# Lightbrite88/Argon_Monte_Carlo

Hardware: AMD Instinct MI355X
Metric: particle-steps/sec (higher is better)
Workload: dtype f64; 1 GPU; cube_1e5; geometry=cube, n_particles=100000, n_per_gpu=100000, parallelism=single GPU

## Files before the change

### argon_monte_carlo_amd/csrc/amc_api.hip

```cpp
#include <memory>
#include <type_traits>

#include "amc_host.h"

int amc_fail(amc_ctx *c, int code, const char *fmt, ...)
{
    char buf[512];
    va_list ap;
    va_start(ap, fmt);
    vsnprintf(buf, sizeof buf, fmt, ap);
    va_end(ap);
    if (c) c->err = buf;
    return code;
}

static thread_local std::string g_create_err;

void amc_prof_begin(amc_ctx *c, int kclass)
{
    if (!c->profiling) return;
    if (c->ev_used == c->ev_pool.size()) {
        hipEvent_t a, b;
        (void)ctx_event(c, &a, hipEventDefault);
        (void)ctx_event(c, &b, hipEventDefault);
// ... 272 lines not shown
    AMC_HIP(c, dalloc(c, &c->d_od, 16));
    AMC_HIP(c, hipMemsetAsync(c->d_od, 0, 16 * sizeof(int), c->stream));
    if (palloc(c, &c->h_pin, (size_t)4 << 20, hipHostMallocDefault) == hipSuccess) c->h_pin_bytes = (size_t)4 << 20;
    return AMC_OK;
}

extern "C" {

int amc_abi_version(void) { return AMC_ABI_VERSION; }

const char *amc_last_error(const amc_ctx *ctx) { return ctx ? ctx->err.c_str() : g_create_err.c_str(); }

const char *amc_kernel_name(int k)
{
    static const char *names[AMC_K_COUNT] = {"drift_walls", "bin_count", "bin_scan",     "bin_scatter", "detect",  "resolve",
                                             "bounds",      "validate",  "resolve_more", "commit",      "clusters_wide", "fixup",
                                             "fields"};
    return (k >= 0 && k < AMC_K_COUNT) ? names[k] : "?";
}

void amc_destroy(amc_ctx *c)
{
    if (!c) return;
    hipSetDevice(c->device);
    hipStreamSynchronize(c->stream);
    ctx_free_since(c, 0);
    delete c;
}

int amc_create(amc_ctx **out, const amc_params *p)
{
    if (!out || !p) { g_create_err = "null argument"; return AMC_ERR_INVALID; }
    *out = nullptr;
    if (p->struct_size != (int32_t)sizeof(amc_params)) {
        g_create_err = "amc_params.struct_size mismatch (ABI)";
        return AMC_ERR_INVALID;
    }
    if (p->n < 0 || p->n > 0x7fffffffLL || !(p->collision_range > 0) || !(p->argon_mass > 0) || p->geometry < 0 ||
        p->geometry > AMC_GEOM_PORE_ENERGISED) {
        g_create_err = "invalid amc_params (n, collision_range, argon_mass or geometry)";
        return AMC_ERR_INVALID;
    }
    int ndev = 0;
    if (hipGetDeviceCount(&ndev) != hipSuccess || ndev <= 0 || p->device < 0 || p->device >= ndev) {
        g_create_err = "no usable HIP device (libargonmc has no CPU fallback)";
        return AMC_ERR_NO_DEVICE;
    }
    amc_ctx *c = new (std::nothrow) amc_ctx();
    if (!c) { g_create_err = "out of host memory"; return AMC_ERR_INVALID; }
    c->P = *p;
    c->device = p->device;
    c->n = p->n; c->hi = p->n;
    c->keep_prior = (p->reserved0 & 1) != 0;
    read_env(c);
    std::unique_ptr<amc_ctx, void (*)(amc_ctx *)> guard(c, [](amc_ctx *x) { g_create_err = x->err; amc_destroy(x); });
    AMC_HIP(c, hipSetDevice(c->device));
    AMC_HIP(c, ctx_stream(c, &c->own_stream));
    c->stream = c->own_stream;
    c->allpairs = (p->geometry == AMC_GEOM_CELL) || (p->detect_mode != 1 && c->n <= c->allpairs_max_n);
    c->detect_ap = c->allpairs || p->detect_mode == 2;
    if (p->geometry == AMC_GEOM_CELL && p->detect_mode == 1) {
        return amc_fail(c, AMC_ERR_INVALID, "AMC_GEOM_CELL has no cell grid: detect_mode must be 0 or 2");
    }
    int rc;
    if ((rc = alloc_state(c)) || (rc = alloc_grid_lists(c)) || (rc = alloc_resolve_ws(c)) || (rc = alloc_outputs(c)) ||
        (rc = alloc_host_words(c)))
        return rc;
    if (c->debug_resolve) {
        AMC_HIP(c, dalloc(c, &c->d_dbg, 128 + 128 * 512));
        AMC_HIP(c, hipMemsetAsync(c->d_dbg, 0, sizeof(long long) * (128 + 128 * 512), c->stream));
        { const long long big = 0x7fffffffffffffffLL; AMC_HIP(c, hipMemcpyAsync(c->d_dbg + 28, &big, sizeof big, hipMemcpyHostToDevice, c->stream)); }
    }
    AMC_HIP(c, hipStreamSynchronize(c->stream));
    *out = guard.release();
    return AMC_OK;
}

int amc_set_stream(amc_ctx *c, void *hip_stream)
{
    if (!c) return AMC_ERR_INVALID;
    hipSetDevice(c->device);
    amc_prof_collect(c);
    if (c->stream) hipStreamSynchronize(c->stream);
    c->stream = hip_stream ? (hipStream_t)hip_stream : c->own_stream;
    return AMC_OK;
}

int amc_use_null_stream(amc_ctx *c)
{
    if (!c) return AMC_ERR_INVALID;
    hipSetDevice(c->device);
    amc_prof_collect(c);
    if (c->stream) hipStreamSynchronize(c->stream);
    c->stream = nullptr;
    return AMC_OK;
}

int amc_synchronize(amc_ctx *c)
{
    if (!c) return AMC_ERR_INVALID;
    AMC_HIP(c, hipSetDevice(c->device));
    AMC_HIP(c, hipStreamSynchronize(c->stream));
    return AMC_OK;
}

int amc_upload(amc_ctx *c, const double *x, const double *y, const double *z, const double *vx, const double *vy,
               const double *vz, const double *dist, const double *dist_x, const double *dist_y, const double *dist_z,
               const uint8_t *full_path)
{
    if (!c) return AMC_ERR_INVALID;
    AMC_HIP(c, hipSetDevice(c->device));
    { int rc_ = amc_flush(c); if (rc_) return rc_; }
    c->step.lists_age = -1;
    const size_t nb = sizeof(double) * (size_t)c->n;
    const double *src[] = {x, y, z, vx, vy, vz, dist, dist_x, dist_y, dist_z};
    double *dst[] = {c->S.x, c->S.y, c->S.z, c->S.vx, c->S.vy, c->S.vz, c->S.d, c->S.dx, c->S.dy, c->S.dz};
    for (int k = 0; k < 10; k++)
        if (src[k] && nb) AMC_HIP(c, hipMemcpyAsync(dst[k], src[k], nb, hipMemcpyHostToDevice, c->stream));
    if (full_path && c->n) AMC_HIP(c, hipMemcpyAsync(c->S.flag, full_path, (size_t)c->n, hipMemcpyHostToDevice, c->stream));
    { int rc_ = amc_publish_velocities(c); if (rc_) return rc_; }
    AMC_HIP(c, hipStreamSynchronize(c->stream));
    c->uploaded = true;
    return AMC_OK;
}

int amc_publish_velocities(amc_ctx *c)
{
    if (!c->kin_vpub || c->n <= 0) return AMC_OK;
    const size_t nb = sizeof(double) * (size_t)c->n;
    const double *src[3] = {c->S.vx, c->S.vy, c->S.vz};
    for (int e = 0; e < 3; e++)
        AMC_HIP(c, hipMemcpyAsync(c->kin_vpub + (size_t)e * (size_t)c->n, src[e], nb, hipMemcpyDeviceToDevice, c->stream));
    return AMC_OK;
}

int amc_download(amc_ctx *c, double *x, double *y, double *z, double *vx, double *vy, double *vz, double *dist,
                 double *dist_x, double *dist_y, double *dist_z, uint8_t *full_path)
{
    if (!c) return AMC_ERR_INVALID;
    AMC_HIP(c, hipSetDevice(c->device));
    { int rc_ = amc_flush(c); if (rc_) return rc_; }
    const size_t nb = sizeof(double) * (size_t)c->n;
    double *dst[] = {x, y, z, vx, vy, vz, dist, dist_x, dist_y, dist_z};
    double *src[] = {c->S.x, c->S.y, c->S.z, c->S.vx, c->S.vy, c->S.vz, c->S.d, c->S.dx, c->S.dy, c->S.dz};
    for (int k = 0; k < 10; k++)
        if (dst[k] && nb) AMC_HIP(c, hipMemcpyAsync(dst[k], src[k], nb, hipMemcpyDeviceToHost, c->stream));
    if (full_path && c->n) AMC_HIP(c, hipMemcpyAsync(full_path, c->S.flag, (size_t)c->n, hipMemcpyDeviceToHost, c->stream));
    AMC_HIP(c, hipStreamSynchronize(c->stream));
    return AMC_OK;
}

int amc_download_prior(amc_ctx *c, double *px, double *py, double *pz)
{
    if (!c) return AMC_ERR_INVALID;
    if (!c->keep_prior) return amc_fail(c, AMC_ERR_STATE, "prior_*_vals are only kept when amc_params.reserved0 bit0 is set");
    AMC_HIP(c, hipSetDevice(c->device));
    const size_t nb = sizeof(double) * (size_t)c->n;
    if (px && nb) AMC_HIP(c, hipMemcpyAsync(px, c->S.px, nb, hipMemcpyDeviceToHost, c->stream));
    if (py && nb) AMC_HIP(c, hipMemcpyAsync(py, c->S.py, nb, hipMemcpyDeviceToHost, c->stream));
    if (pz && nb) AMC_HIP(c, hipMemcpyAsync(pz, c->S.pz, nb, hipMemcpyDeviceToHost, c->stream));
    AMC_HIP(c, hipStreamSynchronize(c->stream));
    return AMC_OK;
}

int amc_paths_pending(amc_ctx *c, size_t *n)
{
    if (!c || !n) return AMC_ERR_INVALID;
    AMC_HIP(c, hipSetDevice(c->device));
    amc_dev_counters now;
    int rc = amc_read_counters(c, &now);
    if (rc) return rc;
    *n = std::min<size_t>(now.path_count, c->out.cap);
    return AMC_OK;
}

int amc_drain_paths(amc_ctx *c, amc_path_record *out, size_t cap, size_t *n)
{
    if (!c || !n) return AMC_ERR_INVALID;
    size_t pending;
    int rc = amc_paths_pending(c, &pending);
    if (rc) return rc;
    if (pending > cap) return amc_fail(c, AMC_ERR_CAPACITY, "amc_drain_paths: %zu records pending, buffer holds %zu", pending, cap);
    if (pending) AMC_HIP(c, hipMemcpyAsync(out, c->d_rec, sizeof(amc_path_record) * pending, hipMemcpyDeviceToHost, c->stream));
    unsigned int zero = 0;
    AMC_HIP(c, hipMemcpyAsync(&c->d_cnt->path_count, &zero, sizeof zero, hipMemcpyHostToDevice, c->stream));
    AMC_HIP(c, hipStreamSynchronize(c->stream));
    *n = pending;
    return AMC_OK;
}

int amc_histograms(amc_ctx *c, uint64_t *counts, uint64_t *n_paths_total)
{
    if (!c) return AMC_ERR_INVALID;
    AMC_HIP(c, hipSetDevice(c->device));
    if (counts) {
        if (!c->d_hist) return amc_fail(c, AMC_ERR_STATE, "histograms disabled (hist_bins == 0)");
    }
    { int rc_ = amc_settle_commit(c); if (rc_) return rc_; }
    std::vector<uint64_t> banks;
    if (counts) {
        banks.resize((size_t)4 * c->out.nbins * AMC_COUNTER_BANKS);
        AMC_HIP(c, hipMemcpyAsync(banks.data(), c->d_hist, sizeof(uint64_t) * banks.size(), hipMemcpyDeviceToHost, c->stream));
    }
    amc_dev_counters now;
    int rc = amc_read_counters(c, &now);
    if (rc) return rc;
    if (counts) {
        const size_t m = (size_t)4 * c->out.nbins;
        for (size_t k = 0; k < m; k++) counts[k] = 0;
        for (int b = 0; b < AMC_COUNTER_BANKS; b++)
            for (size_t k = 0; k < m; k++) counts[k] += banks[(size_t)b * m + k];
    }
    if (n_paths_total) *n_paths_total = now.n_paths_total;
    return AMC_OK;
}

int amc_reset_outputs(amc_ctx *c)
{
    if (!c) return AMC_ERR_INVALID;
    AMC_HIP(c, hipSetDevice(c->device));
    { int rc_ = amc_settle_commit(c); if (rc_) return rc_; }
    if (c->d_hist) AMC_HIP(c, hipMemsetAsync(c->d_hist, 0, sizeof(uint64_t) * 4 * c->out.nbins * AMC_COUNTER_BANKS, c->stream));
    AMC_HIP(c, hipMemsetAsync(c->d_cnt, 0, sizeof(amc_dev_counters), c->stream));
    AMC_HIP(c, hipMemsetAsync(c->d_banks, 0, sizeof(amc_counter_bank) * AMC_COUNTER_BANKS, c->stream));
    AMC_HIP(c, hipStreamSynchronize(c->stream));
    memset(&c->h_prev, 0, sizeof c->h_prev);
    c->out.step = 0;
    return AMC_OK;
}

int amc_pairwise_cell(amc_ctx *c, int64_t n_cell, double *continue_path, double *continue_x_path, double *continue_y_path,
                      double *continue_z_path, uint8_t *has_collided, double *x, double *y, double *z, double *vx,
                      double *vy, double *vz, double *out_paths, size_t cap, size_t *n_paths, int64_t *n_collisions)
{
    if (!c) return AMC_ERR_INVALID;
    if (c->P.geometry != AMC_GEOM_CELL) return amc_fail(c, AMC_ERR_STATE, "amc_pairwise_cell needs an AMC_GEOM_CELL context");
    if (n_cell < 0 || n_cell > c->n) return amc_fail(c, AMC_ERR_INVALID, "n_cell %lld exceeds the context capacity %lld", (long long)n_cell, (long long)c->n);
    AMC_HIP(c, hipSetDevice(c->device));
    const int64_t n_full = c->n;
    c->n = n_cell; c->lo = 0; c->hi = n_cell;
    int rc = amc_upload(c, x, y, z, vx, vy, vz, continue_path, continue_x_path, continue_y_path, continue_z_path, has_collided);
    amc_step_stats st;
    memset(&st, 0, sizeof st);
    size_t pending = 0;
    if (!rc) {
        size_t dummy;
        rc = amc_paths_pending(c, &dummy);
    }
    if (!rc) rc = amc_timestep(c, 0.0, &st);
    if (!rc) rc = amc_download(c, x, y, z, vx, vy, vz, continue_path, continue_x_path, continue_y_path, continue_z_path, has_collided);
    if (!rc) rc = amc_paths_pending(c, &pending);
    if (!rc && pending) {
        std::vector<amc_path_record> rec(pending);
        size_t got = 0;
        rc = amc_drain_paths(c, rec.data(), pending, &got);
        if (!rc) {
            std::sort(rec.begin(), rec.begin() + got, [](const amc_path_record &a, const amc_path_record &b) {
                if (a.step != b.step) return a.step < b.step;
                if (a.i != b.i) return a.i < b.i;
                if (a.j != b.j) return a.j < b.j;
                return a.which < b.which;
            });
            if (got > cap) rc = amc_fail(c, AMC_ERR_CAPACITY, "out_paths holds %zu paths, %zu were completed", cap, got);
            else if (out_paths)
                for (size_t k = 0; k < got; k++) {
                    out_paths[0 * cap + k] = rec[k].total; out_paths[1 * cap + k] = rec[k].px;
                    out_paths[2 * cap + k] = rec[k].py; out_paths[3 * cap + k] = rec[k].pz;
                }
            pending = got;
        }
    }
    if (n_paths) *n_paths = pending;
    if (n_collisions) *n_collisions = st.n_pp;
    c->n = n_full; c->lo = 0; c->hi = n_full;
    return rc;
}

int amc_profile(amc_ctx *c, int enable)
{
    if (!c) return AMC_ERR_INVALID;
    hipSetDevice(c->device);
    amc_prof_collect(c);
    c->profiling = enable != 0;
    return AMC_OK;
}

int amc_overlap_stats(amc_ctx *c, int64_t *out)
{
    if (!c || !out) return AMC_ERR_INVALID;
    AMC_HIP(c, hipSetDevice(c->device));
    amc_dev_counters now;
    int rc = amc_read_counters(c, &now);
    if (rc) return rc;
    out[0] = c->ovl_steps; out[1] = now.n_refiled; out[2] = c->overlap_mode; out[3] = c->max_extra;
    out[4] = c->od_ordered_launches; out[5] = c->od_steps; out[6] = c->od_stalls; out[7] = c->od_stalls_last;
    return AMC_OK;
}

int amc_kernel_times(amc_ctx *c, double *total_ms, int64_t *launches)
{
    if (!c) return AMC_ERR_INVALID;
    hipSetDevice(c->device);
    amc_prof_collect(c);
    if (c->d_dbg) {
        long long h[128];
        hipMemcpy(h, c->d_dbg, sizeof h, hipMemcpyDeviceToHost);
        const double n = h[11] > 0 ? (double)h[11] : 1.0;
        fprintf(stderr, "[amc k_resolve phases, us/launch] count-left %.1f claim %.1f | rounds: collect %.1f pairs %.1f clusters>=3: sort+load %.1f emulate %.1f | overlay %.1f validate %.1f commit %.1f | rounds %.2f cand %.1f complex-members %.2f launches %lld (idle hand-over only %lld)\n",
                h[0] / n / 100.0, h[1] / n / 100.0, h[6] / n / 100.0, h[7] / n / 100.0, h[2] / n / 100.0, h[3] / n / 100.0, h[14] / n / 100.0, h[4] / n / 100.0, h[5] / n / 100.0,
                h[8] / n, h[9] / n, h[10] / n, h[11], h[12]);
        fprintf(stderr, "[amc host candidate count] %d (what the next launch plan is chosen from)\n", c->h_host_ncand ? (int)*c->h_host_ncand : -1);
        if (h[12] > 0)
            fprintf(stderr, "[amc k_resolve idle hand-over, us/launch] entry -> counts read %.2f, -> hand-over written %.2f, -> through the barrier %.2f (%lld launches)\n",
                    h[16] / (double)h[12] / 100.0, h[17] / (double)h[12] / 100.0, h[18] / (double)h[12] / 100.0, h[12]);
        {
            std::vector<long long> wv((size_t)128 * 512);
            hipMemcpy(wv.data(), c->d_dbg + 128, sizeof(long long) * wv.size(), hipMemcpyDeviceToHost);
            long long s[128] = {0}, longest = 0;
            for (int w = 0; w < 512; w++) {
                for (int e = 3; e < 128; e++) if (e != 4) s[e] += wv[(size_t)128 * w + e];
                longest = std::max(longest, wv[(size_t)128 * w + 4]);
            }
            const double nl = h[25] > 0 ? (double)h[25] : 1.0;
            static const char *cn[8] = {"pair", "3-cluster", "4+-cluster", "not owner", "pair+again", "3-cluster+again", "4+-cluster+again", "not owner+again"};
            static const char *pn[12] = {"graph", "walk", "reserve", "small: after emulate", "pair emulate | by the wave: emulate", "publish", "grid probe", "first hop", "particles", "set-up", "overlay probe", "small: prepare"};
            fprintf(stderr, "[amc k_clusters_wide] working waves %lld in %lld launches; launch span (first working wave in -> last out) %.2f us, last out -> ordered workgroup in %.2f us, longest wave ever %.2f us\n",
                    s[3], h[25], h[27] / nl / 100.0, h[26] / nl / 100.0, longest / 100.0);
            fprintf(stderr, "[three-particle path of lane 0] %lld times, %lld continued from the pair's hit; loads + slots %.2f us, emulation %.2f us\n", s[5], s[6],
                    s[7] / (double)std::max<long long>(1, s[5]) / 100.0, s[124] / (double)std::max<long long>(1, s[5]) / 100.0);
            fprintf(stderr, "[pair-wave lifetimes, 2.5 us buckets]");
            for (int k = 0; k < 8; k++) fprintf(stderr, " %lld", s[24 + k]);
            fprintf(stderr, "\n");
            for (int k = 0; k < 8; k++) {
                if (!s[16 + k]) continue;
                fprintf(stderr, "[amc k_clusters_wide %-16s %7lld waves, %5.1f us]", cn[k], s[16 + k], s[8 + k] / (double)s[16 + k] / 100.0);
                for (int e = 0; e < 12; e++) fprintf(stderr, " %s %.2f", pn[e], s[32 + 12 * k + e] / (double)s[16 + k] / 100.0);
                fprintf(stderr, "\n");
            }
        }
    }
    for (int k = 0; k < AMC_K_COUNT; k++) {
        if (total_ms) total_ms[k] = c->k_ms[k];
        if (launches) launches[k] = c->k_launches[k];
    }
    return AMC_OK;
}

}
```

### argon_monte_carlo_amd/csrc/amc_grid.hip

```cpp
#include <stdlib.h>

#include "amc_grid_dev.h"

#define AMC_CR2_INFLATE (1.0 + 1.0e-9)

__global__ __launch_bounds__(256) void k_bin_lists(const double *__restrict__ x, const double *__restrict__ y,
                                                   const double *__restrict__ z, long long n, amc_grid G, amc_lists B,
                                                   amc_dev_counters *cnt, amc_ovl V)
{
    const long long p = (long long)blockIdx.x * blockDim.x + threadIdx.x;
    if (p >= n) return;
    if (V.skip_epoch && (unsigned int)(V.adj_head[p] >> 32) == V.skip_epoch) return;
    bool outside = false;
    amc_list_insert(G, B, (int)p, x[p], y[p], z[p], &outside);
    if (outside) atomicOr(&cnt->flags, 8ULL);
}

struct amc_adj {
    unsigned long long *head;
    int4 *rec;
    int4 *sd;
    int4 *sl_meta;
    int *sl_hits, *ev_gen;
    unsigned int epoch;
    unsigned long long *mark;
};

AMC_DEV int amc_push_candidate(int a, int b, int max_cand, amc_dev_counters *cnt, const amc_adj &D)
{
    const unsigned int k = atomicAdd(&cnt->cand_count, 1u);
    if (k < (unsigned)max_cand) {
        const int hi = a > b ? a : b, lo = a > b ? b : a;
        int4 r;
        r.x = hi; r.y = lo; r.z = -1; r.w = -1;
        if (D.head) {
            const unsigned long long mine = ((unsigned long long)D.epoch << 32) | (unsigned long long)k;
            const unsigned long long oi = atomicExch(&D.head[hi], mine), oj = atomicExch(&D.head[lo], mine);
            r.z = ((unsigned int)(oi >> 32) == D.epoch) ? (int)(unsigned int)(oi & 0xffffffffULL) : -1;
            r.w = ((unsigned int)(oj >> 32) == D.epoch) ? (int)(unsigned int)(oj & 0xffffffffULL) : -1;
            auto mark = [&](int kd) {
                const unsigned long long old = atomicExch(&D.mark[kd], mine);
                if ((unsigned int)(old >> 32) == D.epoch) D.mark[kd] = ((unsigned long long)D.epoch << 32) | AMC_MARK_MULTI;
            };
            if (r.z >= 0) mark(r.z);
            if (r.w >= 0) mark(r.w);
        }
        D.rec[k] = r;
        D.sd[k] = make_int4(-1, -1, 0, 0);
        if (D.head) {
            D.sl_meta[2 * k] = make_int4(-1, 2 * (int)k, 0, 0);
            D.sl_meta[2 * k + 1] = make_int4(-1, 2 * (int)k + 1, 0, 0);
            atomicAnd(&D.sl_hits[2 * k], 0);
            atomicAnd(&D.sl_hits[2 * k + 1], 0);
            *(int4 *)&D.ev_gen[4 * k] = make_int4(0, 0, 0, 0);
        }
        return (int)k;
    }
    atomicOr(&cnt->flags, 1ULL);
    return -1;
}

AMC_DEV void amc_detect_node(const amc_grid &G, const amc_lists &B, int node, double cr2i, double cr_probe, int max_cand,
                             amc_dev_counters *cnt, const amc_adj &D, const int *od_stall = nullptr, int od_tick = 0)
{
    const int stalled = od_stall ? *od_stall : 0;
    amc_rec me_r = B.rec[node];
    const int live = (B.node_of && node < B.n) ? B.node_of[node] : node;
    if (stalled && od_tick > stalled) return;
    if (me_r.x != me_r.x) {
        if (live == node) return;
        node = live;
        me_r = B.rec[node];
        if (me_r.x != me_r.x) return;
    }
    const int me_p = amc_node_particle(B, node);
    double3 me;
    amc_rec_pos(G, me_r, me.x, me.y, me.z);
    auto found_pair = [&](int q) { amc_push_candidate(me_p, amc_node_particle(B, q), max_cand, cnt, D); };
    int q[9];
    q[0] = amc_rec_next(me_r);
    {
        int ocx, ocy, ocz;
        amc_grid_coords(G, me.x, me.y, me.z, ocx, ocy, ocz);
        const int c_own = amc_grid_cell(G, ocx, ocy, ocz, nullptr);
        int c_lo[4], c_hi[4];
        const int nc = amc_grid_box_ranges(G, me.x, me.y, me.z, cr_probe, c_lo, c_hi);
        int cell[8];
#pragma unroll
        for (int k = 0; k < 4; k++)
#pragma unroll
            for (int t = 0; t < 2; t++) {
                const int c = c_lo[k < nc ? k : 0] + t;
                cell[2 * k + t] = (k < nc && c <= c_hi[k < nc ? k : 0] && c < c_own) ? c : -1;
            }
        unsigned long long hv[8];
#pragma unroll
        for (int e = 0; e < 8; e++) hv[e] = (cell[e] >= 0) ? B.head[cell[e]] : 0ULL;
#pragma unroll
        for (int e = 0; e < 8; e++)
            q[1 + e] = (cell[e] >= 0 && (unsigned int)(hv[e] >> 32) == B.epoch) ? (int)(unsigned int)(hv[e] & 0xffffffffULL) : -1;
    }
    for (;;) {
        bool live = false;
#pragma unroll
        for (int e = 0; e < 9; e++) live |= q[e] >= 0;
        if (!live) break;
        amc_rec o[9];
#pragma unroll
        for (int e = 0; e < 9; e++)
            if (q[e] >= 0) o[e] = B.rec[q[e]];
#pragma unroll
        for (int e = 0; e < 9; e++)
            if (q[e] >= 0) {
                double ox, oy, oz;
                amc_rec_pos(G, o[e], ox, oy, oz);
                const double ex = ox - me.x, ey = oy - me.y, ez = oz - me.z;
                if (ex * ex + ey * ey + ez * ez < cr2i) found_pair(q[e]);
                q[e] = amc_rec_next(o[e]);
            }
    }
}

#ifndef AMC_DETECT_MINW
#define AMC_DETECT_MINW 4
#endif
__global__ __launch_bounds__(256, AMC_DETECT_MINW) void k_detect_lists(amc_grid G, amc_lists B, long long n, double cr2i, double cr_probe,
                                                      int max_cand, amc_dev_counters *cnt, amc_adj D, const int *extra_count,
                                                      int max_extra, const int *od_stall, int od_tick, int *wctl_rearm)
{
    const long long nb = (n + blockDim.x - 1) / blockDim.x;
    if ((long long)blockIdx.x < nb) {
        const long long p = (long long)blockIdx.x * blockDim.x + threadIdx.x;
        if (p < n) amc_detect_node(G, B, (int)p, cr2i, cr_probe, max_cand, cnt, D, od_stall, od_tick);
        if (wctl_rearm && p == 0 && !(*od_stall && od_tick > *od_stall)) {
            amc_resolve_ctl *wc = (amc_resolve_ctl *)wctl_rearm;
            for (int b = 0; b < 16; b++) wctl_rearm[32 + b] = 0;
            wc->nslots = 0; wc->nhist = 0; wc->nedges = 0; wc->nfp = 0; wc->ovf = 0; wc->dirty = 0; wc->nclusters = 0;
            wc->changed = 0; wc->active = 0; wc->cur_round = 1;
        }
        return;
    }
    if (!extra_count) return;
    int ne = *extra_count;
    if (ne > max_extra) ne = max_extra;
    const int stride = (int)((gridDim.x - nb) * blockDim.x);
    for (int e = (int)((blockIdx.x - nb) * blockDim.x + threadIdx.x); e < ne; e += stride)
        amc_detect_node(G, B, (int)n + e, cr2i, cr_probe, max_cand, cnt, D, od_stall, od_tick);
}

__global__ __launch_bounds__(256) void k_detect_own(amc_grid G, amc_lists B, long long lo, long long hi, double cr2i,
                                                    double cr_probe, int *__restrict__ out, int cap, amc_dev_counters *cnt)
{
    const long long p = lo + (long long)blockIdx.x * blockDim.x + threadIdx.x;
    if (p >= hi) return;
    amc_rec me_r = B.rec[p];
    const int live = B.node_of ? B.node_of[p] : (int)p;
    if (me_r.x != me_r.x) {
        if (live == (int)p) return;
        me_r = B.rec[live];
        if (me_r.x != me_r.x) return;
    }
    double3 me;
    amc_rec_pos(G, me_r, me.x, me.y, me.z);
    int c_lo[4], c_hi[4];
    const int nc = amc_grid_box_ranges(G, me.x, me.y, me.z, cr_probe, c_lo, c_hi);
    int q[8];
    unsigned long long hv[8];
#pragma unroll
    for (int k = 0; k < 4; k++)
#pragma unroll
        for (int t = 0; t < 2; t++) {
            const int c = c_lo[k < nc ? k : 0] + t;
            const bool on = k < nc && c <= c_hi[k < nc ? k : 0];
            hv[2 * k + t] = on ? B.head[c] : 0ULL;
            q[2 * k + t] = on ? 0 : -1;
        }
#pragma unroll
    for (int e = 0; e < 8; e++)
        q[e] = (q[e] == 0 && (unsigned int)(hv[e] >> 32) == B.epoch) ? (int)(unsigned int)(hv[e] & 0xffffffffULL) : -1;
    for (;;) {
        bool live = false;
#pragma unroll
        for (int e = 0; e < 8; e++) live |= q[e] >= 0;
        if (!live) break;
        amc_rec o[8];
#pragma unroll
        for (int e = 0; e < 8; e++)
            if (q[e] >= 0) o[e] = B.rec[q[e]];
#pragma unroll
        for (int e = 0; e < 8; e++)
            if (q[e] >= 0) {
                double ox, oy, oz;
                amc_rec_pos(G, o[e], ox, oy, oz);
                const double ex = ox - me.x, ey = oy - me.y, ez = oz - me.z;
                const int pq = amc_node_particle(B, q[e]);
                if (pq < (int)p && ex * ex + ey * ey + ez * ez < cr2i) {
                    const int k = atomicAdd(&out[0], 1);
                    if (k < cap) { out[2 + 2 * k] = (int)p; out[3 + 2 * k] = pq; }
                    else atomicOr(&cnt->flags, 1ULL);
                }
                q[e] = amc_rec_next(o[e]);
            }
    }
}

__global__ __launch_bounds__(256) void k_ingest_candidates(const int *__restrict__ blocks, int world, int block_ints, int cap,
                                                           int max_cand, amc_dev_counters *cnt, amc_adj D, int *__restrict__ own)
{
    const int gtid = blockIdx.x * blockDim.x + threadIdx.x, gstride = gridDim.x * blockDim.x;
    for (int r = 0; r < world; r++) {
        const int *b = blocks + (size_t)r * block_ints;
        int nr = b[0];
        if (nr > cap) {
            nr = cap;
            if (gtid == 0) atomicOr(&cnt->flags, 1ULL);
        }
        for (int k = gtid; k < nr; k += gstride) amc_push_candidate(b[2 + 2 * k], b[3 + 2 * k], max_cand, cnt, D);
    }
    if (gtid == 0) own[0] = 0;
}

#define AP_T 256
__global__ __launch_bounds__(AP_T) void k_detect_allpairs(const double *__restrict__ x, const double *__restrict__ y,
                                                          const double *__restrict__ z, int n, int ntiles, double cr2i,
                                                          int max_cand, amc_dev_counters *cnt, amc_adj D)
{
    int bi = (int)((sqrt(8.0 * (double)blockIdx.x + 1.0) - 1.0) * 0.5);
    while ((long long)(bi + 1) * (bi + 2) / 2 <= (long long)blockIdx.x) bi++;
    while ((long long)bi * (bi + 1) / 2 > (long long)blockIdx.x) bi--;
    const int bj = (int)(blockIdx.x - (long long)bi * (bi + 1) / 2);
    if (bi >= ntiles) return;
    __shared__ double tx[AP_T], ty[AP_T], tz[AP_T];
    const int j0 = bj * AP_T;
    const int jj = j0 + threadIdx.x;
    tx[threadIdx.x] = (jj < n) ? x[jj] : 0.0;
    ty[threadIdx.x] = (jj < n) ? y[jj] : 0.0;
    tz[threadIdx.x] = (jj < n) ? z[jj] : 0.0;
    __syncthreads();
    const int i = bi * AP_T + threadIdx.x;
    if (i >= n) return;
    const double xi = x[i], yi = y[i], zi = z[i];
    int jmax = n - j0;
    if (jmax > AP_T) jmax = AP_T;
    if (bi == bj && jmax > (int)threadIdx.x) jmax = threadIdx.x;
#pragma unroll 4
    for (int k = 0; k < jmax; k++) {
        const double ex = tx[k] - xi, ey = ty[k] - yi, ez = tz[k] - zi;
        const double d2 = fma(ez, ez, fma(ey, ey, ex * ex));
        if (d2 < cr2i) amc_push_candidate(i, j0 + k, max_cand, cnt, D);
    }
}

hipError_t amc_launch_bin(amc_ctx *c)
{
    if (c->allpairs || c->n <= 0) return hipSuccess;
    const long long n = c->n;
    c->B.epoch++;
    c->step.lists_age = -1;
    amc_prof_begin(c, AMC_K_BIN_COUNT);
    amc_ovl V;
    V.adj_head = nullptr; V.skip_epoch = 0;
    AMC_LAUNCH(c, k_bin_lists, dim3((unsigned)((n + 255) / 256)), dim3(256), c->S.x, c->S.y, c->S.z, n,
                       c->G, c->B, c->d_cnt, V);
    amc_prof_end(c);
    return hipGetLastError();
}

hipError_t amc_launch_bin_ovl(amc_ctx *c, int to, unsigned int skip_epoch, hipStream_t stream)
{
    const long long n = c->n;
    amc_ovl V;
    V.adj_head = c->W.adj_head; V.skip_epoch = skip_epoch;
    amc_prof_begin(c, AMC_K_BIN_COUNT);
    AMC_LAUNCH_ON(c, stream, k_bin_lists, dim3((unsigned)((n + 255) / 256)), dim3(256), c->S_buf[to].x, c->S_buf[to].y, c->S_buf[to].z, n,
                  c->G, c->B_buf[to], c->d_cnt, V);
    amc_prof_end(c);
    return hipGetLastError();
}

#define AP2_T 1024
#define AP2_R 4
#define AP2_THREADS (AP2_T / AP2_R)
#define AP2_CHUNK 8
__global__ __launch_bounds__(AP2_THREADS) void k_detect_allpairs_tiled(const double *__restrict__ x, const double *__restrict__ y,
                                                               const double *__restrict__ z, int n, int ntiles, double thr,
                                                               double ox, double oy, double oz,
                                                               int max_cand, amc_dev_counters *cnt, amc_adj D)
{
    int bi = (int)((sqrt(8.0 * (double)blockIdx.x + 1.0) - 1.0) * 0.5);
    while ((long long)(bi + 1) * (bi + 2) / 2 <= (long long)blockIdx.x) bi++;
    while ((long long)bi * (bi + 1) / 2 > (long long)blockIdx.x) bi--;
    const int bj = (int)(blockIdx.x - (long long)bi * (bi + 1) / 2);
    if (bi >= ntiles) return;
    __shared__ double tx[AP2_T], ty[AP2_T], tz[AP2_T], tn[AP2_T];
    const int j0 = bj * AP2_T;
    for (int t = threadIdx.x; t < AP2_T; t += AP2_THREADS) {
        const int jj = j0 + t;
        const bool in = jj < n;
        const double X = in ? x[jj] - ox : 0.0, Y = in ? y[jj] - oy : 0.0, Z = in ? z[jj] - oz : 0.0;
        tx[t] = X; ty[t] = Y; tz[t] = Z;
        tn[t] = in ? fma(Z, Z, fma(Y, Y, X * X)) : 1.0e300;
    }
    __syncthreads();
    int ii[AP2_R];
    double ax[AP2_R], ay[AP2_R], az[AP2_R], ti[AP2_R];
#pragma unroll
    for (int r = 0; r < AP2_R; r++) {
        ii[r] = bi * AP2_T + r * AP2_THREADS + (int)threadIdx.x;
        const bool in = ii[r] < n;
        const double X = in ? x[ii[r]] - ox : 0.0, Y = in ? y[ii[r]] - oy : 0.0, Z = in ? z[ii[r]] - oz : 0.0;
        ax[r] = -2.0 * X; ay[r] = -2.0 * Y; az[r] = -2.0 * Z;
        ti[r] = in ? thr - fma(Z, Z, fma(Y, Y, X * X)) : -1.0e300;
    }
    const bool diag = bi == bj;
    for (int k0 = 0; k0 < AP2_T; k0 += AP2_CHUNK) {
        bool any = false;
#pragma unroll
        for (int u = 0; u < AP2_CHUNK; u++) {
            const double jx = tx[k0 + u], jy = ty[k0 + u], jz = tz[k0 + u], jn = tn[k0 + u];
#pragma unroll
            for (int r = 0; r < AP2_R; r++) any |= fma(az[r], jz, fma(ay[r], jy, fma(ax[r], jx, jn))) < ti[r];
        }
        if (any) {
            for (int u = 0; u < AP2_CHUNK; u++) {
                const int j = j0 + k0 + u;
                const double jx = tx[k0 + u], jy = ty[k0 + u], jz = tz[k0 + u], jn = tn[k0 + u];
#pragma unroll
                for (int r = 0; r < AP2_R; r++)
                    if (fma(az[r], jz, fma(ay[r], jy, fma(ax[r], jx, jn))) < ti[r] && (diag ? j < ii[r] : true))
                        amc_push_candidate(ii[r], j, max_cand, cnt, D);
            }
        }
    }
}

static unsigned int next_sweep_epoch(unsigned int epoch)
{
    epoch = (epoch + 1u) & 0x3fffffffu;
    return epoch ? epoch : 1u;
}

hipError_t amc_launch_detect(amc_ctx *c)
{
    const long long n = c->n;
    if (n <= 0) return hipSuccess;
    const double cr2i = c->allpairs || c->detect_ap ? c->P.collision_range * c->P.collision_range * AMC_CR2_INFLATE : c->G.cr2_probe;
    amc_adj D;
    c->step.sweep_epoch = next_sweep_epoch(c->step.sweep_epoch);
    c->step.plan_split = !c->allpairs && !(c->h_host_ncand && *c->h_host_ncand <= c->plan_small);
    D.head = c->allpairs ? nullptr : c->W.adj_head; D.rec = c->W.cand4; D.sd = c->W.cand_s; D.epoch = c->step.sweep_epoch;
    D.sl_meta = c->W.sl_meta; D.sl_hits = c->W.sl_hits; D.ev_gen = c->W.ev_gen; D.mark = c->W.cand_mark;
    amc_prof_begin(c, AMC_K_DETECT);
    if (c->detect_ap) {
        if (n >= 16 * AP2_T && c->G.ncells > 0) {
            const int ntiles = (int)((n + AP2_T - 1) / AP2_T);
            const long long nblocks = (long long)ntiles * (ntiles + 1) / 2;
            const double ex = c->G.gx * c->G.h, ey = c->G.gy * c->G.h, ez = c->G.gz * c->G.h;
            const double thr = cr2i + 64.0 * 1.1102230246251565e-16 * (ex * ex + ey * ey + ez * ez);
            AMC_LAUNCH(c, k_detect_allpairs_tiled, dim3((unsigned)nblocks), dim3(AP2_THREADS), c->S.x, c->S.y,
                               c->S.z, (int)n, ntiles, thr, c->G.x0, c->G.y0, c->G.z0, c->W.max_cand, c->d_cnt, D);
        } else {
            const int ntiles = (int)((n + AP_T - 1) / AP_T);
            const long long nblocks = (long long)ntiles * (ntiles + 1) / 2;
            if (nblocks > 0)
                AMC_LAUNCH(c, k_detect_allpairs, dim3((unsigned)nblocks), dim3(AP_T), c->S.x, c->S.y,
                                   c->S.z, (int)n, ntiles, cr2i, c->W.max_cand, c->d_cnt, D);
        }
    } else {
        const bool extras = c->B.extra != nullptr && c->keep_K < 2;
        const int slot = (c->B.extra == c->extra_buf[1]) ? 1 : 0;
        const int bs = c->detect_bs;
        AMC_LAUNCH(c, k_detect_lists, dim3((unsigned)((n + bs - 1) / bs) + (extras ? 4u : 0u)), dim3(bs), c->G, c->B, n, cr2i,
                   c->G.cr_probe, c->W.max_cand, c->d_cnt, D, (const int *)(extras ? c->extra_count + slot : nullptr),
                   c->max_extra, (const int *)(c->od_active ? c->d_od : nullptr), c->od_tick,
                   (c->od_active && !c->step.od_prev_ordered) ? c->W.wctl : nullptr);
    }
    amc_prof_end(c);
    return hipGetLastError();
}

hipError_t amc_launch_detect_own(amc_ctx *c)
{
    const long long cnt = c->hi - c->lo;
    amc_prof_begin(c, AMC_K_DETECT);
    if (cnt > 0)
        AMC_LAUNCH(c, k_detect_own, dim3((unsigned)((cnt + 255) / 256)), dim3(256), c->G, c->B, (long long)c->lo, (long long)c->hi,
                   c->G.cr2_probe, c->G.cr_probe, c->cand_send, c->cand_cap, c->d_cnt);
    amc_prof_end(c);
    return hipGetLastError();
}

hipError_t amc_launch_ingest(amc_ctx *c, int world)
{
    amc_adj D;
    c->step.sweep_epoch = next_sweep_epoch(c->step.sweep_epoch);
    c->step.plan_split = !(c->h_host_ncand && *c->h_host_ncand <= c->plan_small);
    D.head = c->W.adj_head; D.rec = c->W.cand4; D.sd = c->W.cand_s; D.epoch = c->step.sweep_epoch;
    D.sl_meta = c->W.sl_meta; D.sl_hits = c->W.sl_hits; D.ev_gen = c->W.ev_gen; D.mark = c->W.cand_mark;
    amc_prof_begin(c, AMC_K_DETECT);
    AMC_LAUNCH(c, k_ingest_candidates, dim3(16), dim3(256), (const int *)c->cand_recv, world, 2 + 2 * c->cand_cap, c->cand_cap,
               c->W.max_cand, c->d_cnt, D, c->cand_send);
    amc_prof_end(c);
    return hipGetLastError();
}
```

### argon_monte_carlo_amd/csrc/amc_internal.h

```cpp
#pragma once
#include <hip/hip_runtime.h>
#include <hip/hip_ext.h>
#include <stdint.h>

#include <string>
#include <vector>

#include "amc_device.h"

#define RS_SLOT_DOUBLES 12

struct amc_state {
    double *x, *y, *z, *vx, *vy, *vz, *d, *dx, *dy, *dz;
    double *px, *py, *pz;
    uint8_t *flag;
};

struct amc_grid {
    double x0, y0, z0, h;
    double inv_h;
    int uniform;
    int gx, gy, gz;
    int ncells;
    double cr_probe;
    double cr2_probe;
    const int *lay_lo;
    const int *lay_n;
    const int *lay_off;
};

struct amc_rec {
    float x, y, z;
    int next;
};
#define AMC_MARK_MULTI 0xffffffffu
struct amc_lists {
    unsigned long long *head;
    amc_rec *rec;
    unsigned int epoch;
    int n;
    int *extra;
    int *cell_of;
    int *node_of;
    int *wave_count;
    int wave_cap;
};
#define AMC_LIST_KEEP_DEFAULT_PORE 4
#define AMC_EXTRA_NODES(n) ((int)std::min<long long>(std::max<long long>(4096, (long long)(n) / 64), 1 << 22))

struct amc_ovl {
    const unsigned long long *adj_head;
    unsigned int skip_epoch;
};

struct amc_lazy {
    int *slot_of;
    const double *state;
    const uint8_t *moved;
    int enabled;
};

struct amc_resolve_ctl {
    int nslots, nedges, nhist, nev, dirty, changed, nhits, nfp, ovf, nclusters, ncomplex;
    int rounds, ncand, active, ok, edges_done;
    int lazy_ns, nslots0, hist_begin, cur_round;
};
struct rs_event {
    int phase, i, j, which;
    long long cell;
    int slot, pad;
    double val[4];
};
struct amc_resolve_ws {
    int4 *cand4, *cand_s;
    unsigned long long *cand_mark;
    int max_cand;
    unsigned long long *adj_head;
    int *slot_of;
    unsigned int *victim;
    int max_slots;
    int4 *sl_meta;
    int *sl_hits;
    uint8_t *sl_moved;
    double *sl_state;
    int *edge_a, *edge_b;
    int max_edges;
    double4 *hist;
    int max_hist;
    int *ov_head, *ov_next;
    int *ev_gen;
    rs_event *ev;
    int *ctl;
    int *wctl;
    int *raise_dev, *raise_host;
    int raise_tick;
    int *sl_label, *sl_tmp;
    uint8_t *sl_dirty;
    unsigned long long *sl_key;
    int *order;
    double *cw_d[10];
    int *cw_tmp, *cw_pidx, *cw_slot;
    uint8_t *cw_flag, *cw_moved;
};

struct amc_temp_ws {
    int *idx, *count;
    double *t, *contact, *normal, *dir, *Es, *dpz, *dE;
    unsigned char *ok;
    int *h_idx, *h_count;
    double *h_contact, *h_normal, *h_dir, *h_Es, *h_dpz, *h_dE;
    void *pin;
    int cap;
    int last_case = -1, last_n = 0;
    int pre_case = -1;
    std::vector<int> perm;
    int *def_idx;
    double *def_dir, *def_Es, *def_dpz, *def_dE;
    double *h_def_Es, *h_def_dpz, *h_def_dE;
    int def_case = -1, def_n = 0;
    std::vector<int> def_perm;
};

struct temp_dev_segments {
    int *idx, *count;
    double *t, *contact, *normal, *dir, *Es, *dpz, *dE;
    unsigned char *ok;
    int cap;
};
struct amc_temp_pass {
    amc_temp_rng g;
    temp_dev_segments D;
};
struct amc_temp_row {
    double sums[3];
    unsigned int had;
    unsigned int pad;
};
struct amc_temp_dev_ws {
    int *idx, *count;
    double *t, *contact, *normal, *dir, *Es, *dpz, *dE;
    unsigned char *ok;
    int cap;
    amc_temp_row *series;
    int64_t series_cap, series_n;
    int *perm;
    int *ovf;
    amc_temp_pass *pass;
    bool fetched;
    int h_count[7];
    std::vector<int> h_idx[7];
    std::vector<double> h_dpz[7], h_dE[7];
    std::vector<unsigned char> h_ok[7];
};

struct amc_fields_ws {
    bool on;
    amc_field_grid g;
    int bins;
    double w[3];
    int max_blocks;
    int blocks_env;
    unsigned long long *slab;
    unsigned long long *tot;
    unsigned long long *meta;
};

enum amc_res_kind { AMC_RES_DEVICE, AMC_RES_PINNED, AMC_RES_STREAM, AMC_RES_EVENT };
struct amc_res { void *p; amc_res_kind kind; };

#define AMC_OD_AHEAD 2
#define AMC_OD_MAX_N 100000
#define AMC_OD_RING 64
#define AMC_OD_MIN_STEPS 8
#define AMC_PLAN_SMALL 430

struct amc_step_state {
    bool lazy_pending;
    bool commit_pending;
    bool commit_defer;
    int commit_step = 0;
    unsigned int sweep_epoch;
    bool plan_split;
    int lists_age = -1;
    int lists_owner;
    bool od_prev_ordered = true;
};

struct amc_ctx {
    amc_params P;
    int device;
    hipStream_t own_stream, stream;
    std::string err;
    int64_t n, lo, hi;
    bool uploaded;
    bool keep_prior;
    std::vector<amc_res> owned;
    amc_step_state step;
    amc_state S;
    char *s_slab;
    amc_grid G;
    std::vector<int> h_lay_lo, h_lay_n, h_lay_off;
    int *d_lay;
    amc_lists B;
    int max_extra;
    int keep_K;
    size_t keep_pool;
    bool allpairs;
    bool detect_ap;
    amc_resolve_ws W;
    char *w_slab;
    volatile int *h_host_ncand;
    int *d_host_ncand;
    amc_temp_ws T;
    amc_temp_dev_ws TD;
    amc_fields_ws F;
    amc_out out;
    amc_path_record *d_rec;
    unsigned long long *d_hist;
    double *d_edges;
    amc_dev_counters *d_cnt;
    amc_counter_bank *d_banks;
    amc_dev_counters h_prev;
    long long *d_dbg;
    char *h_pin;
    size_t h_pin_bytes;
    int overlap_mode;
    bool overlap_split;
    int cw_blocks_env;
    int stream_bs;
    int detect_bs;
    bool temp_unfused;
    bool temp_run_unfused;
    bool ordered_always;
    int64_t od_max_n = AMC_OD_MAX_N;
    int od_ahead = AMC_OD_AHEAD;
    int plan_small = AMC_PLAN_SMALL;
    long long allpairs_max_n;
    int list_keep;
    int max_hist_env;
    bool debug_resolve;
    bool profiling;
    double k_ms[AMC_K_COUNT];
    int64_t k_launches[AMC_K_COUNT];
    std::vector<std::pair<hipEvent_t, hipEvent_t>> ev_pool;
    std::vector<std::pair<int, int>> ev_pending;
    size_t ev_used;
    hipEvent_t prof_ev0, prof_ev1;
    amc_state S_buf[2];
    char *s_slab2;
    amc_lists B_buf[2];
    int *extra_buf[2];
    int *extra_count;
    amc_wev wev_buf[2];
    hipStream_t stream2;
    hipEvent_t ev_detect, ev_stream;
    unsigned int *ovl_flags;
    unsigned int ovl_tick;
    int ovl_sync_values;
    int64_t ovl_steps;
    int *d_od;
    volatile int *h_od_stall, *h_od_done;
    int *d_od_stall_host, *d_od_done_host;
    bool od_active;
    int od_tick = 1;
    int od_handled;
    int64_t od_ordered_launches;
    int64_t od_steps;
    int64_t od_stalls, od_stalls_last;
    bool mg_count_pp = true;
    double *kin_send, *kin_recv;
    double *kin_vpub;
    int kin_world;
    int64_t kin_m, kin_cap, kin_block;
    int *cand_send, *cand_recv;
    int cand_cap, cand_world;
    int *mg_wave_count;
    int mg_waves_pack, mg_waves_unpack;
    bool mg_keep;
    int kin_mode = 1;
    bool kin_lists;
    bool kin_counts_clear;
};

int amc_fail(amc_ctx *c, int code, const char *fmt, ...);
#define AMC_HIP(c, call)                                                                                      \
    do {                                                                                                      \
        hipError_t e__ = (call);                                                                              \
        if (e__ != hipSuccess) return amc_fail((c), AMC_ERR_HIP, "%s failed: %s (%s:%d)", #call,             \
                                               hipGetErrorString(e__), __FILE__, __LINE__);                   \
    } while (0)

#define AMC_LAUNCH(c, kernel, grid, block, ...) \
    hipExtLaunchKernelGGL(kernel, grid, block, 0, (c)->stream, (c)->prof_ev0, (c)->prof_ev1, 0, __VA_ARGS__)
#define AMC_LAUNCH_ON(c, stream_, kernel, grid, block, ...) \
    hipExtLaunchKernelGGL(kernel, grid, block, 0, stream_, (c)->prof_ev0, (c)->prof_ev1, 0, __VA_ARGS__)

void amc_prof_begin(amc_ctx *c, int kclass);
void amc_prof_end(amc_ctx *c);
void amc_prof_cancel(amc_ctx *c);
void amc_prof_collect(amc_ctx *c);

#define AMC_ST_DRIFT 1
#define AMC_ST_WALLS 2
#define AMC_ST_BOUNDS 4
#define AMC_ST_BOUNDS_PRE 8
#define AMC_TEMP_RUN_FUSED_DEFAULT 1
#define AMC_ST_TEMP_CASES 16
static inline int amc_step_stages(int geometry, bool prev_bounds = false)
{
    if (geometry == AMC_GEOM_CUBE) return AMC_ST_DRIFT | AMC_ST_WALLS;
    return AMC_ST_DRIFT | AMC_ST_WALLS | AMC_ST_BOUNDS | (prev_bounds && geometry == AMC_GEOM_PORE ? AMC_ST_BOUNDS_PRE : 0);
}

hipError_t amc_launch_stream(amc_ctx *c, double dt, int stages, int bounds_slot, bool fuse_bin = false);
hipError_t amc_launch_stream_ovl(amc_ctx *c, double dt, int stages, int from, unsigned int skip_epoch, hipStream_t stream,
                                 bool build_lists = true);
hipError_t amc_launch_fixup(amc_ctx *c, double dt, int stages, int from, unsigned int sweep_epoch);
hipError_t amc_launch_bin_ovl(amc_ctx *c, int to, unsigned int skip_epoch, hipStream_t stream);
int amc_list_build_mode(amc_ctx *c, int owner, bool kept);
hipError_t amc_launch_bin(amc_ctx *c);
hipError_t amc_launch_detect(amc_ctx *c);
hipError_t amc_launch_detect_own(amc_ctx *c);
hipError_t amc_launch_ingest(amc_ctx *c, int world);
hipError_t amc_launch_resolve(amc_ctx *c, bool defer_commit = false);
struct rs_args;
hipError_t amc_launch_wide_only(amc_ctx *c, rs_args *used);
hipError_t amc_launch_ordered(amc_ctx *c, const rs_args &used);
hipError_t amc_launch_apply(amc_ctx *c);
hipError_t amc_launch_commit(amc_ctx *c);
struct amc_commit_args;
amc_commit_args amc_make_commit_args(amc_ctx *c);
hipError_t amc_launch_temp_hits(amc_ctx *c, int case_id);
hipError_t amc_launch_temp_apply(amc_ctx *c, int case_id, int n, bool park = false);
hipError_t amc_launch_temp_velocity(amc_ctx *c, int case_id, int n);
hipError_t amc_launch_temp_cases_device(amc_ctx *c, const amc_temp_rng *cfg);
hipError_t amc_launch_temp_sums(amc_ctx *c, int64_t row);
temp_dev_segments amc_temp_segments(amc_ctx *c);
hipError_t amc_launch_kin_pack(amc_ctx *c, int world, int rank, int unpack);
int amc_kin_banks(void);
```

Measured before the change: 2.298 billion particle-steps/s.

## Aggregate candidate-slot atomics per wavefront in collision detection

Collision detection is split into a first walk that records up to two hits per node, one wavefront-wide atomicAdd on the candidate counter using ballot/popcount to assign slots, and a second full walk only for nodes with more than two hits. The first neighbour record of the node's own cell list is also loaded early to overlap with the head loads. The aim is to cut contention on the global candidate counter. In exchange, nodes with three or more hits walk their neighbours twice, and all lanes now enter detect_node so the ballot sees the whole wavefront. Optional timestamp instrumentation is added behind a compile flag.

```diff
diff --git a/argon_monte_carlo_amd/csrc/amc_api.hip b/argon_monte_carlo_amd/csrc/amc_api.hip
--- a/argon_monte_carlo_amd/csrc/amc_api.hip
+++ b/argon_monte_carlo_amd/csrc/amc_api.hip
@@ -598,6 +598,9 @@
     if (!c) return AMC_ERR_INVALID;
     hipSetDevice(c->device);
     amc_prof_collect(c);
+#ifdef AMC_DETECT_STAMPS
+    amc_detect_stamps_print(stderr);
+#endif
     if (c->d_dbg) {
         long long h[128];
         hipMemcpy(h, c->d_dbg, sizeof h, hipMemcpyDeviceToHost);
diff --git a/argon_monte_carlo_amd/csrc/amc_grid.hip b/argon_monte_carlo_amd/csrc/amc_grid.hip
--- a/argon_monte_carlo_amd/csrc/amc_grid.hip
+++ b/argon_monte_carlo_amd/csrc/amc_grid.hip
@@ -3,6 +3,30 @@
 #include "amc_grid_dev.h"
 
 #define AMC_CR2_INFLATE (1.0 + 1.0e-9)
+
+#ifdef AMC_DETECT_STAMPS
+#define AMC_STAMP_ROWS (1 << 17)
+__device__ unsigned int amc_stamp_rows[AMC_STAMP_ROWS][8];
+__device__ unsigned int amc_stamp_count;
+#define AMC_DETECT_STAMP(st, i)                                                                                        \
+    do {                                                                                                               \
+        if (st) { asm volatile("s_waitcnt vmcnt(0)" ::: "memory"); (st)[i] = (unsigned int)wall_clock64(); }           \
+    } while (0)
+void amc_detect_stamps_print(FILE *f)
+{
+    static unsigned int rows[AMC_STAMP_ROWS][8];
+    unsigned int nr = 0;
+    if (hipMemcpyFromSymbol(&nr, HIP_SYMBOL(amc_stamp_count), sizeof nr) != hipSuccess) return;
+    const unsigned int kept = nr < AMC_STAMP_ROWS ? nr : AMC_STAMP_ROWS;
+    if (hipMemcpyFromSymbol(rows, HIP_SYMBOL(amc_stamp_rows), sizeof(unsigned int) * 8 * kept) != hipSuccess) return;
+    fprintf(f, "[amc detect stamps] %u rows (%u kept): epoch, 6 stamps (10 ns ticks), hits\n", nr, kept);
+    for (unsigned int r = 0; r < kept; r++)
+        fprintf(f, "[amc detect stamp] %u %u %u %u %u %u %u %u\n", rows[r][0], rows[r][1], rows[r][2], rows[r][3], rows[r][4],
+                rows[r][5], rows[r][6], rows[r][7]);
+}
+#else
+#define AMC_DETECT_STAMP(st, i) do { } while (0)
+#endif
 
 __global__ __launch_bounds__(256) void k_bin_lists(const double *__restrict__ x, const double *__restrict__ y,
                                                    const double *__restrict__ z, long long n, amc_grid G, amc_lists B,
@@ -26,9 +50,9 @@
     unsigned long long *mark;
 };
 
-AMC_DEV int amc_push_candidate(int a, int b, int max_cand, amc_dev_counters *cnt, const amc_adj &D)
-{
-    const unsigned int k = atomicAdd(&cnt->cand_count, 1u);
+AMC_DEV int amc_store_candidate(unsigned int k, int a, int b, int max_cand, amc_dev_counters *cnt, const amc_adj &D,
+                                unsigned int *stamps = nullptr)
+{
     if (k < (unsigned)max_cand) {
         const int hi = a > b ? a : b, lo = a > b ? b : a;
         int4 r;
@@ -38,6 +62,7 @@
             const unsigned long long oi = atomicExch(&D.head[hi], mine), oj = atomicExch(&D.head[lo], mine);
             r.z = ((unsigned int)(oi >> 32) == D.epoch) ? (int)(unsigned int)(oi & 0xffffffffULL) : -1;
             r.w = ((unsigned int)(oj >> 32) == D.epoch) ? (int)(unsigned int)(oj & 0xffffffffULL) : -1;
+            AMC_DETECT_STAMP(stamps, 5);
             auto mark = [&](int kd) {
                 const unsigned long long old = atomicExch(&D.mark[kd], mine);
                 if ((unsigned int)(old >> 32) == D.epoch) D.mark[kd] = ((unsigned long long)D.epoch << 32) | AMC_MARK_MULTI;
@@ -60,26 +85,53 @@
     return -1;
 }
 
-AMC_DEV void amc_detect_node(const amc_grid &G, const amc_lists &B, int node, double cr2i, double cr_probe, int max_cand,
-                             amc_dev_counters *cnt, const amc_adj &D, const int *od_stall = nullptr, int od_tick = 0)
+AMC_DEV int amc_push_candidate(int a, int b, int max_cand, amc_dev_counters *cnt, const amc_adj &D)
+{
+    return amc_store_candidate(atomicAdd(&cnt->cand_count, 1u), a, b, max_cand, cnt, D);
+}
+
+
+AMC_DEV bool amc_detect_start(const amc_lists &B, int &node, amc_rec &me_r, const int *od_stall, int od_tick)
 {
     const int stalled = od_stall ? *od_stall : 0;
-    amc_rec me_r = B.rec[node];
+    me_r = B.rec[node];
     const int live = (B.node_of && node < B.n) ? B.node_of[node] : node;
-    if (stalled && od_tick > stalled) return;
+    if (stalled && od_tick > stalled) return false;
     if (me_r.x != me_r.x) {
-        if (live == node) return;
+        if (live == node) return false;
         node = live;
         me_r = B.rec[node];
-        if (me_r.x != me_r.x) return;
-    }
-    const int me_p = amc_node_particle(B, node);
+        if (me_r.x != me_r.x) return false;
+    }
+    return true;
+}
+
+template <bool REST>
+AMC_DEV void amc_detect_walk(const amc_grid &G, const amc_lists &B, int node, const amc_rec &me_r, double cr2i, double cr_probe,
+                             int &h1, int &h2, bool &more, int max_cand, amc_dev_counters *cnt, const amc_adj &D,
+                             unsigned int *stamps = nullptr)
+{
     double3 me;
     amc_rec_pos(G, me_r, me.x, me.y, me.z);
-    auto found_pair = [&](int q) { amc_push_candidate(me_p, amc_node_particle(B, q), max_cand, cnt, D); };
+    auto visit = [&](int qn, const amc_rec &o) {
+        double ox, oy, oz;
+        amc_rec_pos(G, o, ox, oy, oz);
+        const double ex = ox - me.x, ey = oy - me.y, ez = oz - me.z;
+        const bool hit = ex * ex + ey * ey + ez * ez < cr2i;
+        if (REST) {
+            if (hit && qn != h1 && qn != h2)
+                amc_push_candidate(amc_node_particle(B, node), amc_node_particle(B, qn), max_cand, cnt, D);
+        } else {
+            more |= hit && h2 >= 0;
+            h2 = (hit && h1 >= 0 && h2 < 0) ? qn : h2;
+            h1 = (hit && h1 < 0) ? qn : h1;
+        }
+    };
     int q[9];
     q[0] = amc_rec_next(me_r);
     {
+        amc_rec o0 = me_r;
+        if (q[0] >= 0) o0 = B.rec[q[0]];
         int ocx, ocy, ocz;
         amc_grid_coords(G, me.x, me.y, me.z, ocx, ocy, ocz);
         const int c_own = amc_grid_cell(G, ocx, ocy, ocz, nullptr);
@@ -99,7 +151,12 @@
 #pragma unroll
         for (int e = 0; e < 8; e++)
             q[1 + e] = (cell[e] >= 0 && (unsigned int)(hv[e] >> 32) == B.epoch) ? (int)(unsigned int)(hv[e] & 0xffffffffULL) : -1;
-    }
+        if (q[0] >= 0) {
+            visit(q[0], o0);
+            q[0] = amc_rec_next(o0);
+        }
+    }
+    AMC_DETECT_STAMP(stamps, 2);
     for (;;) {
         bool live = false;
 #pragma unroll
@@ -112,13 +169,58 @@
 #pragma unroll
         for (int e = 0; e < 9; e++)
             if (q[e] >= 0) {
-                double ox, oy, oz;
-                amc_rec_pos(G, o[e], ox, oy, oz);
-                const double ex = ox - me.x, ey = oy - me.y, ez = oz - me.z;
-                if (ex * ex + ey * ey + ez * ez < cr2i) found_pair(q[e]);
+                visit(q[e], o[e]);
                 q[e] = amc_rec_next(o[e]);
             }
     }
+}
+
+AMC_DEV void amc_push_hits(const amc_lists &B, int node, int h1, int h2, int max_cand, amc_dev_counters *cnt, const amc_adj &D,
+                           unsigned int *stamps = nullptr)
+{
+    const unsigned long long m1 = __ballot(h1 >= 0), m2 = __ballot(h2 >= 0);
+    if (h1 < 0) return;
+    const unsigned long long below = (1ULL << __lane_id()) - 1ULL;
+    const int n1 = __popcll(m1);
+    unsigned int base = 0;
+    if ((m1 & below) == 0ULL) base = atomicAdd(&cnt->cand_count, (unsigned int)(n1 + __popcll(m2)));
+    base = __builtin_amdgcn_readfirstlane(base);
+    AMC_DETECT_STAMP(stamps, 4);
+    const int me_p = amc_node_particle(B, node);
+    amc_store_candidate(base + (unsigned int)__popcll(m1 & below), me_p, amc_node_particle(B, h1), max_cand, cnt, D, stamps);
+    if (h2 >= 0)
+        amc_store_candidate(base + (unsigned int)(n1 + __popcll(m2 & below)), me_p, amc_node_particle(B, h2), max_cand, cnt, D);
+#ifdef AMC_DETECT_STAMPS
+    if ((m1 & below) == 0ULL) {
+        const unsigned int row = atomicAdd(&amc_stamp_count, 1u);
+        if (row < AMC_STAMP_ROWS) {
+            amc_stamp_rows[row][0] = D.epoch;
+            for (int e = 0; e < 6; e++) amc_stamp_rows[row][1 + e] = stamps[e];
+            amc_stamp_rows[row][7] = (unsigned int)(n1 + __popcll(m2));
+        }
+    }
+#endif
+}
+
+AMC_DEV void amc_detect_node(const amc_grid &G, const amc_lists &B, bool active, int node, double cr2i, double cr_probe, int max_cand,
+                             amc_dev_counters *cnt, const amc_adj &D, const int *od_stall = nullptr, int od_tick = 0)
+{
+#ifdef AMC_DETECT_STAMPS
+    unsigned int stamp_words[6] = {0, 0, 0, 0, 0, 0};
+    unsigned int *stamps = stamp_words;
+#else
+    unsigned int *stamps = nullptr;
+#endif
+    AMC_DETECT_STAMP(stamps, 0);
+    int h1 = -1, h2 = -1;
+    bool more = false;
+    amc_rec me_r;
+    if (active) active = amc_detect_start(B, node, me_r, od_stall, od_tick);
+    AMC_DETECT_STAMP(stamps, 1);
+    if (active) amc_detect_walk<false>(G, B, node, me_r, cr2i, cr_probe, h1, h2, more, max_cand, cnt, D, stamps);
+    AMC_DETECT_STAMP(stamps, 3);
+    amc_push_hits(B, node, h1, h2, max_cand, cnt, D, stamps);
+    if (more) amc_detect_walk<true>(G, B, node, B.rec[node], cr2i, cr_probe, h1, h2, more, max_cand, cnt, D);
 }
 
 #ifndef AMC_DETECT_MINW
@@ -131,7 +233,7 @@
     const long long nb = (n + blockDim.x - 1) / blockDim.x;
     if ((long long)blockIdx.x < nb) {
         const long long p = (long long)blockIdx.x * blockDim.x + threadIdx.x;
-        if (p < n) amc_detect_node(G, B, (int)p, cr2i, cr_probe, max_cand, cnt, D, od_stall, od_tick);
+        amc_detect_node(G, B, p < n, (int)p, cr2i, cr_probe, max_cand, cnt, D, od_stall, od_tick);
         if (wctl_rearm && p == 0 && !(*od_stall && od_tick > *od_stall)) {
             amc_resolve_ctl *wc = (amc_resolve_ctl *)wctl_rearm;
             for (int b = 0; b < 16; b++) wctl_rearm[32 + b] = 0;
@@ -144,8 +246,10 @@
     int ne = *extra_count;
     if (ne > max_extra) ne = max_extra;
     const int stride = (int)((gridDim.x - nb) * blockDim.x);
-    for (int e = (int)((blockIdx.x - nb) * blockDim.x + threadIdx.x); e < ne; e += stride)
-        amc_detect_node(G, B, (int)n + e, cr2i, cr_probe, max_cand, cnt, D, od_stall, od_tick);
+    for (int e0 = (int)((blockIdx.x - nb) * blockDim.x); e0 < ne; e0 += stride) {
+        const int e = e0 + (int)threadIdx.x;
+        amc_detect_node(G, B, e < ne, (int)n + e, cr2i, cr_probe, max_cand, cnt, D, od_stall, od_tick);
+    }
 }
 
 __global__ __launch_bounds__(256) void k_detect_own(amc_grid G, amc_lists B, long long lo, long long hi, double cr2i,
diff --git a/argon_monte_carlo_amd/csrc/amc_internal.h b/argon_monte_carlo_amd/csrc/amc_internal.h
--- a/argon_monte_carlo_amd/csrc/amc_internal.h
+++ b/argon_monte_carlo_amd/csrc/amc_internal.h
@@ -319,6 +319,9 @@
 hipError_t amc_launch_bin_ovl(amc_ctx *c, int to, unsigned int skip_epoch, hipStream_t stream);
 int amc_list_build_mode(amc_ctx *c, int owner, bool kept);
 hipError_t amc_launch_bin(amc_ctx *c);
+#ifdef AMC_DETECT_STAMPS
+void amc_detect_stamps_print(FILE *f);
+#endif
 hipError_t amc_launch_detect(amc_ctx *c);
 hipError_t amc_launch_detect_own(amc_ctx *c);
 hipError_t amc_launch_ingest(amc_ctx *c, int world);
```

Measured after the change: 2.287 billion particle-steps/s. Within noise of the previous version (-0.5%).
